# MILAB-IIT-CV/ATDN_vSLAM

Hardware: AMD Instinct MI355X
Metric: frame-pairs/sec, KITTI 1241x376 odometry inference at 1/2/4/8 MI355X (higher is better)
Workload: dtype f32 via 3xf16 split MFMA (fp32 accumulate); 1 GPU; KITTI seq-03-shaped 376x1241 uint8 frames (resident in HBM) resized to 376x1232, GMA flow 12 GRU iters + CLVO head -> 6-DoF trajectory (BASELINE configs[1]); streams_per_gpu=2, gru_iters=12, parallelism=pairs sharded x1, one all-gather of 512-d features, replicated LSTM scan

## Files before the change

atdn_vslam_amd/_lib.py:

```python
import ctypes as C
import os

_HERE = os.path.dirname(os.path.abspath(__file__))
LIB_PATH = os.environ.get("ATDN_LIB_PATH") or os.path.join(_HERE, "libatdn_hip.so")

_f32p = C.POINTER(C.c_float)
_i64p = C.POINTER(C.c_int64)
_vp = C.c_void_p

SIGNATURES = {
    "atdn_version": (C.c_int, []),
    "atdn_last_error": (C.c_char_p, []),
    "atdn_gma_create": (C.c_int, [C.POINTER(_vp), C.c_int, C.c_int, C.c_int, C.c_int]),
    "atdn_gma_set_low_latency": (C.c_int, [_vp, C.c_int]),
    "atdn_gma_load": (C.c_int, [_vp, C.c_char_p, _vp, _i64p, C.c_int]),
    "atdn_gma_finalize": (C.c_int, [_vp]),
    "atdn_gma_forward": (C.c_int, [_vp, _vp, _vp, C.c_int, C.c_int, _vp, _vp, _vp, _vp]),
    "atdn_gma_forward_predictions": (C.c_int, [_vp, _vp, _vp, C.c_int, C.c_int, _vp, _vp, _vp]),
    "atdn_gma_forward_sequence": (C.c_int, [_vp, _vp, C.c_int, C.c_int, _vp, _vp, _vp, _vp]),
    "atdn_gma_forward_sequence_continued": (C.c_int, [_vp, _vp, C.c_int, C.c_int, _vp, _vp, _vp, _vp]),
    "atdn_gma_debug_read": (C.c_long, [_vp, C.c_char_p, _vp, C.c_long, _vp]),
    "atdn_gma_profile": (C.c_int, [_vp, C.c_int, C.c_int, C.c_int, _f32p, _vp]),
    "atdn_gma_profile_mode": (C.c_int, [_vp, C.c_int, C.c_int, C.c_int, C.c_int, _f32p, _vp]),
    "atdn_gma_set_range_probe": (C.c_int, [_vp, C.c_int]),
# ... 45 lines not shown
    "atdn_flow_two_view_depth": (C.c_int, [_vp, _vp, _vp, C.c_int, C.c_int, C.c_int, C.c_double, C.c_double, C.c_double, C.c_double,
                                           C.c_double, C.c_double, C.c_double, _vp, _vp, _vp]),
    "atdn_flow_two_view_depth_host": (C.c_int, [_vp, _vp, _vp, C.c_int, C.c_int, C.c_int, C.c_double, C.c_double, C.c_double,
                                                C.c_double, C.c_double, C.c_double, C.c_double, _vp, _vp]),
    "atdn_depth_backproject": (C.c_int, [_vp, C.c_int, C.c_int, C.c_int, C.c_double, C.c_double, C.c_double, C.c_double, _vp, _vp]),
    "atdn_flow_track_step": (C.c_int, [_vp, _vp, _vp, _vp, C.c_int, C.c_int, C.c_int, _vp, _vp, _vp, C.c_double, C.c_double, C.c_double,
                                       C.c_double, C.c_double, C.c_double, C.c_double, _vp, _vp, _vp]),
    "atdn_flow_track_step_host": (C.c_int, [_vp, _vp, _vp, _vp, C.c_int, C.c_int, C.c_int, _vp, _vp, _vp, C.c_double, C.c_double,
                                            C.c_double, C.c_double, C.c_double, C.c_double, C.c_double, _vp, _vp]),
    "atdn_map_search": (C.c_int, [_vp, C.c_int, C.c_int, _vp, C.c_int, C.c_int, _vp, _vp, _vp]),
    "atdn_map_gather_images_u8": (C.c_int, [_vp, C.c_int, C.c_long, _vp, C.c_int, _vp, _vp]),
    "atdn_corr_lookup": (C.c_int, [_vp, _vp, _vp, _vp, C.c_int, C.c_int, C.c_int, _vp, _vp, C.c_int, _vp]),
    "atdn_corr_pyramid": (C.c_int, [_vp, _vp, C.c_int, C.c_int, C.c_int, C.c_int, _vp, _vp, _vp, _vp, _vp]),
    "atdn_corr_lookup_bricks": (C.c_int, [_vp, _vp, C.c_int, C.c_int, C.c_int, C.c_int, _vp, _vp, _vp, _vp, _vp, _vp, _vp, _vp,
                                          _vp, _vp]),
    "atdn_conv2d_nhwc": (C.c_int, [_vp, C.c_int, C.c_int, C.c_int, C.c_int, _vp, _vp, C.c_int, C.c_int, C.c_int,
                                   C.c_int, C.c_int, C.c_int, C.c_int, _vp, _vp]),
    "atdn_conv2d_nhwc_sf": (C.c_int, [_vp, C.c_int, C.c_int, C.c_int, C.c_int, _vp, _vp, C.c_int, C.c_int, C.c_int,
                                      C.c_int, C.c_int, C.c_int, _vp, _vp]),
    "atdn_conv2d_nhwc_sf_epi": (C.c_int, [_vp, C.c_int, C.c_int, C.c_int, C.c_int, _vp, _vp, C.c_int, C.c_int, C.c_int,
                                      C.c_int, C.c_int, C.c_int, C.c_int, _vp, _vp]),
}

GMA_STAGES = ("fnet", "corr", "pool", "cnet", "attention", "lookup", "motion_encoder", "aggregate", "gru_zr", "gru_q",
              "flow_head", "mask", "gru_ctx", "attn_logits", "agg_vt", "convc1", "gru_zr_v", "gru_q_v")

_lib = None


def lib():
# ... 37 lines not shown
```

atdn_vslam_amd/csrc/capi.hip:

```cpp
#include "../../include/atdn_hip.h"

#include <cmath>
#include <cstring>

#include "clvo.h"
#include "gma.h"
#include "vae.h"
#include "clvo_train.h"
#include "train_kernels.h"
#include "frontend.h"
#include "conv_sf.h"
#include "epilogues_sf.h"
#include "flow_args.h"
#include "flow_consistency_host.h"
#include "flow_track_host.h"
#include "two_view_host.h"
#include "warm_start_host.h"

namespace atdn {
extern template TileChoice conv_dispatch<MODE_TAP, EpiBias<ACT_NONE>>(const ConvShape&, EpiBias<ACT_NONE>, hipStream_t);
extern template TileChoice conv_dispatch<MODE_TAP, EpiBias<ACT_RELU>>(const ConvShape&, EpiBias<ACT_RELU>, hipStream_t);
extern template TileChoice conv_dispatch<MODE_ROW, EpiBias<ACT_NONE>>(const ConvShape&, EpiBias<ACT_NONE>, hipStream_t);
extern template TileChoice conv_dispatch<MODE_ROW, EpiBias<ACT_RELU>>(const ConvShape&, EpiBias<ACT_RELU>, hipStream_t);
extern template TileChoice conv_dispatch<MODE_TAP, EpiScale>(const ConvShape&, EpiScale, hipStream_t);
// ... 429 lines not shown
  bp.N = N; bp.NPB = brick_pixel_blocks(N);
  DeviceBuf f1, f2, plain[3], fbrick[4], pyr[4], scratch, outsf;
  DeviceBuf* all[] = {&f1, &f2, &plain[0], &plain[1], &plain[2], &fbrick[0], &fbrick[1], &fbrick[2], &fbrick[3],
                      &pyr[0], &pyr[1], &pyr[2], &pyr[3], &scratch, &outsf};
  WeightArena A;
  try {
    sf_counter_attach();
    f1.alloc(n8 * 256); f2.alloc(n8 * 256);
    launch_to_sf(fmap1, f1.p, n8, 256, st);
    launch_to_sf(fmap2, f2.p, n8, 256, st);
    float* rowmajor[4] = {pyr0, pyr1, pyr2, pyr3};
    int pH[4], pW[4];
    for (int l = 0; l < 4; ++l) {
      pH[l] = H8 >> l; pW[l] = W8 >> l;
      bp.H[l] = pH[l]; bp.W[l] = pW[l]; bp.BW[l] = cdiv(pW[l], 8); bp.BH[l] = cdiv(pH[l], 4); bp.NB[l] = bp.BW[l] * bp.BH[l] * 32;
      const float* src = f2.p;
      long src_sb = (long)N * 256;
      if (l > 0) {
        const float* prev = l == 1 ? f2.p : plain[l - 2].p;
        const long prev_sb = l == 1 ? (long)N * 256 : (long)pH[l - 1] * pW[l - 1] * 256;
        src_sb = (long)pH[l] * pW[l] * 256;
        plain[l - 1].alloc((long)B * src_sb);
        launch_pool_features_sf(prev, B, pH[l - 1], pW[l - 1], 256, prev_sb, plain[l - 1].p, src_sb, st);
        src = plain[l - 1].p;
      }
      fbrick[l].alloc((long)B * bp.NB[l] * 256);
      launch_brick_rows(src, src_sb, B, pH[l], pW[l], 256, fbrick[l].p, (long)bp.NB[l] * 256, st);
      pyr[l].alloc((long)B * bp.NPB * kBrickPixelBlock * bp.NB[l]);
      launch_corr_bricks(f1.p, (long)N * 256, fbrick[l].p, (long)bp.NB[l] * 256, B, N, bp.NB[l], 1.0f / sqrtf(256.0f), pyr[l].p, false, st);
      bp.base[l] = pyr[l].p;
      if (rowmajor[l]) launch_unbrick(pyr[l].p, bp.NB[l], N, pH[l], pW[l], n8, rowmajor[l], st);
    }
    if (samples) {
      outsf.alloc(n8 * 352);
      launch_lookup_bricks(bp, coords, n8, outsf.p, st);
      scratch.alloc(n8 * 352);
      launch_from_sf(outsf.p, scratch.p, n8, 352, st);
      ATDN_HIP(hipMemcpy2DAsync(samples, 324 * sizeof(float), scratch.p, 352 * sizeof(float), 324 * sizeof(float), (size_t)n8,
                                hipMemcpyDeviceToDevice, st));
    }
    if (cor1) {
      StateDict sd;
// ... 10 lines not shown
        launch_lookup_conv(bp, coords, n8, nullptr, L.wf16, L.wscale, L.b, csf.p, false, st);
        launch_from_sf(csf.p, cor1, n8, 256, st);
        ATDN_HIP(hipStreamSynchronize(st));
      } catch (...) { csf.release(); throw; }
      csf.release();
    }
    ATDN_HIP(hipStreamSynchronize(st));
  } catch (...) {
    (void)hipDeviceSynchronize();
    for (auto* b : all) b->release();
    A.release();
    throw;
  }
  for (auto* b : all) b->release();
  A.release();
  ATDN_API_END
}

int atdn_conv2d_nhwc(const float* src, int nimg, int H, int W, int Cin, const float* weight_host,
                     const float* bias_host, int Cout, int KH, int KW, int stride, int padH, int padW, int relu,
                     float* dst, void* stream) {
  ATDN_API_BEGIN
  ATDN_CHECK(src && weight_host && dst && nimg >= 1, "null argument");
  const bool row = (Cin == 4 || Cin == 16);
  ATDN_CHECK(row || Cin % 32 == 0, "Cin must be 4, 16 or a multiple of 32");
  StateDict sd;
  const int64_t ws[4] = {Cout, Cin, KH, KW};
  sd.put("c.weight", weight_host, ws, 4);
  std::vector<float> zb(Cout, 0.f);
  const int64_t bs[1] = {Cout};
// ... 136 lines not shown
```

atdn_vslam_amd/csrc/gma.h:

```cpp
#pragma once
#include <vector>
#include <map>
#include <memory>

#include "attention.h"
#include "conv_dispatch.h"
#include "kernels.h"
#include "range_probe.h"
#include "weights.h"

namespace atdn {

struct EncoderWeights {
  PackedConv stem;
  struct Block { PackedConv c1, c2, ds; bool has_ds = false; } blk[6];
  PackedConv head;
};

class DeviceBuf {
 public:
  float* p = nullptr;
  long n = 0;
  void alloc(long count) {
    n = count;
// ... 74 lines not shown
  WeightArena arena_;
  bool ready_ = false;
  bool use_graph_ = true;
  EncoderWeights fnet_, cnet_;
  PackedConv convc1_, convc2_, convf1_, convf2_, convm_, to_v_, to_qk_;
  long convf1_sf_off_ = -1;
  float convf1_wscale_ = 1.f;
  float fh2_mul_ = 1.f;
  long fh2_w32_off_ = -1;
  DeviceBuf fhG_;
  PackedConv gru_zr_[2], gru_q_[2], fh1_, fh2_, mask0_, mask2_;
  PackedConv gru_zr_ctx_[2], gru_q_ctx_[2];
  const float* gamma_ = nullptr;
  long gamma_off_ = -1;

  DeviceBuf img4_, enc_[4], scratch_, pcnt_, fin_, fmap_, psum_, pm2_, mean_[3], rstd_[3];
  DeviceBuf pyr_[4], h_[2], x_, qk_, attn_, vT_, corrfeat_, cor1_, corflo_, flo1_, z_, rh_, fh_, mask_;
  DeviceBuf coords1_, flow4_, pre_zr_[2], pre_q_[2];
  int pyrH_[4], pyrW_[4];
  size_t ws_bytes_ = 0;

  struct Timer;
  Timer* timer_ = nullptr;
  void mark(int stage, hipStream_t st);

  hipStream_t cap_stream_ = nullptr;
  std::map<std::pair<int, int>, hipGraphExec_t> graphs_;
};

}
```

atdn_vslam_amd/csrc/gma.hip:

```cpp
#include "gma.h"
#include "small_convs.h"
#include "conv_sf.h"
#include "epilogues_sf.h"

namespace atdn { const float* zero_line(); }

namespace atdn {

extern template TileChoice conv_dispatch<MODE_TAP, EpiBias<ACT_NONE>>(const ConvShape&, EpiBias<ACT_NONE>, hipStream_t);
extern template TileChoice conv_dispatch<MODE_TAP, EpiBias<ACT_RELU>>(const ConvShape&, EpiBias<ACT_RELU>, hipStream_t);
extern template TileChoice conv_dispatch<MODE_ROW, EpiBias<ACT_RELU>>(const ConvShape&, EpiBias<ACT_RELU>, hipStream_t);
extern template TileChoice conv_dispatch<MODE_TAP, EpiBiasStats>(const ConvShape&, EpiBiasStats, hipStream_t);
extern template TileChoice conv_dispatch<MODE_ROW, EpiBiasStats>(const ConvShape&, EpiBiasStats, hipStream_t);
extern template TileChoice conv_dispatch<MODE_TAP, EpiBiasReluAddRelu>(const ConvShape&, EpiBiasReluAddRelu, hipStream_t);
extern template TileChoice conv_dispatch<MODE_TAP, EpiContextSplit>(const ConvShape&, EpiContextSplit, hipStream_t);
extern template TileChoice conv_dispatch<MODE_TAP, EpiScale>(const ConvShape&, EpiScale, hipStream_t);
extern template TileChoice conv_dispatch<MODE_TAP, EpiQK>(const ConvShape&, EpiQK, hipStream_t);
extern template TileChoice conv_dispatch<MODE_TAP, EpiStoreT>(const ConvShape&, EpiStoreT, hipStream_t);
extern template TileChoice conv_dispatch<MODE_TAP, EpiAggregate>(const ConvShape&, EpiAggregate, hipStream_t);
extern template TileChoice conv_dispatch<MODE_TAP, EpiGruZR>(const ConvShape&, EpiGruZR, hipStream_t);
extern template TileChoice conv_dispatch<MODE_TAP, EpiGruQ>(const ConvShape&, EpiGruQ, hipStream_t);
extern template TileChoice conv_dispatch<MODE_TAP, EpiFlowDelta>(const ConvShape&, EpiFlowDelta, hipStream_t);

extern template TileChoice conv_dispatch<MODE_ROW, SfBias<ACT_RELU>>(const ConvShape&, SfBias<ACT_RELU>, hipStream_t);
// ... 125 lines not shown
  ATDN_HIP(hipStreamWaitEvent(to, e, 0));
}

void GmaNet::set_low_latency(bool on) {
  ATDN_CHECK(!ready_, "set_low_latency: call it before finalize() (the workspace and the captured graphs depend on it)");
  low_latency_ = on;
}

GmaNet::~GmaNet() {
  DeviceGuard dg(dev_);
  (void)hipDeviceSynchronize();
  for (auto& kv : graphs_) (void)hipGraphExecDestroy(kv.second);
  if (cap_stream_) (void)hipStreamDestroy(cap_stream_);
  if (par_stream_) (void)hipStreamDestroy(par_stream_);
  for (auto& e : par_events_) (void)hipEventDestroy(e);
  DeviceBuf* all[] = {&img4_, &enc_[0], &enc_[1], &enc_[2], &enc_[3], &scratch_, &pcnt_, &fin_, &fmap_, &psum_, &pm2_, &mean_[0], &mean_[1], &mean_[2], &rstd_[0],
                      &rstd_[1], &rstd_[2], &pyr_[0], &pyr_[1], &pyr_[2], &pyr_[3], &h_[0], &h_[1], &x_, &qk_, &attn_, &vT_,
                      &corrfeat_, &cor1_, &corflo_, &flo1_, &z_, &rh_, &fh_, &mask_, &coords1_, &flow4_, &pre_zr_[0],
                      &pre_zr_[1], &pre_q_[0], &pre_q_[1], &rowmax_, &rinv_,
                      &fbrick_[0], &fbrick_[1], &fbrick_[2], &fbrick_[3], &fplain_[0], &fplain_[1], &fplain_[2], &coords_used_, &fhG_,
                      &attn_part_, &enc2_[0], &enc2_[1], &enc2_[2], &enc2_[3]};
  for (auto* b : all) b->release();
  if (probe_slots_) (void)hipFree(probe_slots_);
  arena_.release();
}

void GmaNet::set_probe(bool on) {
  ATDN_CHECK(!on || precision == 0,
             "the range probe needs an exact-fp32 handle (ATDN_PRECISION_F32): only that path writes every intermediate tensor "
             "as plain fp32 and never clamps; the split-f16 / f16 paths store range-limited values and fuse some tensors away");
  probe_ = on;
// ... 104 lines not shown
  resolve_encoder(arena_, fnet_);
  resolve_encoder(arena_, cnet_);
  for (PackedConv* L : {&convc1_, &convc2_, &convf1_, &convf2_, &convm_, &to_v_, &to_qk_, &gru_zr_[0], &gru_zr_[1],
                        &gru_q_[0], &gru_q_[1], &fh1_, &fh2_, &mask0_, &mask2_})
    resolve(arena_, *L);
  if (sf) for (PackedConv* L : {&gru_zr_ctx_[0], &gru_zr_ctx_[1], &gru_q_ctx_[0], &gru_q_ctx_[1]}) resolve(arena_, *L);
  gamma_ = arena_.dev(gamma_off_);

  const int B = maxB;
  const int H2 = conv_out(H, 7, 2, 3), W2 = conv_out(W, 7, 2, 3);
  const long n8 = (long)B * N;
  img4_.alloc(2L * B * H * W * 4);
  for (int i = 0; i < (sf ? 4 : 3); ++i) enc_[i].alloc(2L * B * H2 * W2 * 64);
  fmap_.alloc(2L * B * N * 256);
  const long groups = (long)cdiv(H2 * W2, 64) * 4 + 8;
  psum_.alloc(2L * B * groups * 128); pm2_.alloc(2L * B * groups * 128); pcnt_.alloc(2L * B * groups); fin_.alloc(2L * B * 32 * 128 * 4 * 2);
  for (int i = 0; i < 3; ++i) { mean_[i].alloc(2L * B * 128); rstd_[i].alloc(2L * B * 128); }
  pyrH_[0] = H8; pyrW_[0] = W8;
  for (int l = 1; l < 4; ++l) { pyrH_[l] = pyrH_[l - 1] / 2; pyrW_[l] = pyrW_[l - 1] / 2; }
  ATDN_CHECK(pyrH_[3] >= 2 && pyrW_[3] >= 2, "frame too small for a 4-level pyramid");
  for (int l = 0; l < 4; ++l) {
    brickBW_[l] = cdiv(pyrW_[l], 8); brickBH_[l] = cdiv(pyrH_[l], 4); brickNB_[l] = brickBW_[l] * brickBH_[l] * 32;
    pyr_[l].alloc(classic_ ? n8 * pyrH_[l] * pyrW_[l] : (long)B * brick_pixel_blocks(N) * kBrickPixelBlock * brickNB_[l]);
  }
  if (sf) {
    for (int l = 0; l < 4; ++l) fbrick_[l].alloc((long)B * brickNB_[l] * 256);
    for (int l = 1; l < 4; ++l) fplain_[l - 1].alloc((long)B * pyrH_[l] * pyrW_[l] * 256);
    coords_used_.alloc(n8 * 2);
  }
  h_[0].alloc(n8 * 128); h_[1].alloc(n8 * 128); x_.alloc(n8 * XLD);
  const AttnGeom ag = attn_geom(B, N, ldN);
// ... 28 lines not shown
}

void GmaNet::run_encoder(const EncoderWeights& E, bool instance, int nimg, hipStream_t st, float** out_buf, int* outH,
                         int* outW) {
  int h = conv_out(H, 7, 2, 3), w = conv_out(W, 7, 2, 3);
  float* P = enc_[0].p; float* Q = enc_[1].p; float* R = enc_[2].p;
  auto stats_conv = [&](auto mode_tag, const PackedConv& L, const float* src, int ld, int ih, int iw, int stride,
                        int pad, float* dst, int slot) {
    constexpr int MODE = decltype(mode_tag)::value;
    ConvShape s = conv_shape(L, src, ld, (long)ih * iw * ld, nimg, ih, iw, stride, pad, pad);
    const int oh = conv_out(ih, L.KH, stride, pad), ow = conv_out(iw, L.KW, stride, pad);
    EpiBiasStats ep{L.b, dst, (long)oh * ow * L.N, L.N, psum_.p, pm2_.p, 0};
    TileChoice t = conv_dispatch<MODE>(s, ep, st);
    const int groups = cdiv(oh * ow, t.BM) * (t.BM / 32);
    ATDN_CHECK((long)nimg * groups * L.N <= psum_.n, "statistics scratch too small");
    launch_in_finalize_cnt(psum_.p, pm2_.p, nullptr, nimg, groups, oh * ow, L.N, 1e-5f, mean_[slot].p, rstd_[slot].p,
                           reinterpret_cast<double*>(fin_.p), st);
  };
  using TapT = std::integral_constant<int, MODE_TAP>;
  using RowT = std::integral_constant<int, MODE_ROW>;
  auto pr = [&](int bi, const char* leaf, bool limited, const float* p, long pixels, int ch) {
    if (!probe_) return;
    std::string name = instance ? "fnet." : "cnet.";
    if (bi >= 0) name += "layer" + std::to_string(bi / 2 + 1) + "." + std::to_string(bi % 2);
    probe(name + leaf, limited, p, (long)nimg * pixels, ch, ch, st);
  };

  if (instance) {
    stats_conv(RowT{}, E.stem, img4_.p, 4, H, W, 2, 3, P, 0);
    pr(-1, "conv1.raw", false, P, (long)h * w, 64);
    launch_in_apply(P, mean_[0].p, rstd_[0].p, nullptr, nullptr, nullptr, nimg, (long)h * w, 64, st);
  } else {
// ... 183 lines not shown
  const float* images = img4_.p + (long)first_img * H * W * 4;
  int h = conv_out(H, 7, 2, 3), w = conv_out(W, 7, 2, 3);
  DeviceBuf* eb = bufs ? bufs : enc_;
  float* X = eb[0].p; float* R = eb[1].p; float* Y = eb[2].p; float* O = eb[3].p;
  auto stats_sf = [&](const PackedConv& L, const float* src, int ld, int ih, int iw, int stride, int pad, float* dst,
                      int slot, int in_slot = -1) {
    ConvShape s = conv_shape(L, src, ld, (long)ih * iw * ld, nimg, ih, iw, stride, pad, pad);
    if (in_slot >= 0) { s.in_mean = mean_[in_slot].p; s.in_rstd = rstd_[in_slot].p; }
    const int oh = conv_out(ih, L.KH, stride, pad), ow = conv_out(iw, L.KW, stride, pad);
    EpiBiasStats ep{L.b, dst, (long)oh * ow * L.N, L.N, psum_.p, pm2_.p, 0, pcnt_.p};
    TileChoice t = conv_sf_dispatch(s, L.wscale, ep, st);
    const int groups = t.groups_per_img;
    ATDN_CHECK((long)nimg * groups * L.N <= psum_.n && (long)nimg * groups <= pcnt_.n, "statistics scratch too small");
    if (t.counted)
      launch_in_finalize_cnt(psum_.p, pm2_.p, pcnt_.p, nimg, groups, oh * ow, L.N, 1e-5f, mean_[slot].p,
                             rstd_[slot].p, reinterpret_cast<double*>(fin_.p), st);
    else
      launch_in_finalize_cnt(psum_.p, pm2_.p, nullptr, nimg, groups, oh * ow, L.N, 1e-5f, mean_[slot].p, rstd_[slot].p,
                             reinterpret_cast<double*>(fin_.p), st);
  };
  const bool stem_raw = instance && norm_on_load_;
  if (stem_raw) {
    const int groups = stem_sf_groups(h, w);
    ATDN_CHECK((long)nimg * groups * 64 <= psum_.n && (long)nimg * groups <= pcnt_.n, "statistics scratch too small");
    launch_stem_sf(3, images, nimg, H, W, E.stem.wf, E.stem.wscale, E.stem.b, X, psum_.p, pm2_.p, pcnt_.p, nullptr, nullptr, st);
    launch_in_finalize_cnt(psum_.p, pm2_.p, pcnt_.p, nimg, groups, h * w, 64, 1e-5f, mean_[2].p, rstd_[2].p,
                           reinterpret_cast<double*>(fin_.p), st);
  } else if (instance) {
    const int groups = stem_sf_groups(h, w);
    ATDN_CHECK((long)nimg * groups * 64 <= psum_.n && (long)nimg * groups <= pcnt_.n, "statistics scratch too small");
    launch_stem_sf(1, images, nimg, H, W, E.stem.wf, E.stem.wscale, E.stem.b, nullptr, psum_.p, pm2_.p, pcnt_.p, nullptr,
                   nullptr, st);
    launch_in_finalize_cnt(psum_.p, pm2_.p, pcnt_.p, nimg, groups, h * w, 64, 1e-5f, mean_[0].p, rstd_[0].p,
                           reinterpret_cast<double*>(fin_.p), st);
    launch_stem_sf(2, images, nimg, H, W, E.stem.wf, E.stem.wscale, E.stem.b, X, nullptr, nullptr, nullptr, mean_[0].p,
                   rstd_[0].p, st);
  } else {
    launch_stem_sf(0, images, nimg, H, W, E.stem.wf, E.stem.wscale, E.stem.b, X, nullptr, nullptr, nullptr, nullptr,
                   nullptr, st);
  }
  int c = 64;
  for (int bi = 0; bi < 6; ++bi) {
    const auto& Bk = E.blk[bi];
    const int stride = Bk.has_ds ? 2 : 1;
    const int co = Bk.c1.N;
    const int oh = conv_out(h, 3, stride, 1), ow = conv_out(w, 3, stride, 1);
    const long ohw = (long)oh * ow;
    if (instance && norm_on_load_) {
      const bool raw_in = stem_raw && bi == 0;
// ... 93 lines not shown
}

void GmaNet::run_body_sf(int B, int iters, hipStream_t st) {
  float* f;
  const int nfeat = seq_ == 0 ? 2 * B : seq_ == 1 ? B + 1 : B;
  hipStream_t sB = par_ ? par_stream_ : st;
  if (par_) fork(st, sB);
  run_encoder_sf(fnet_, true, nfeat, st, &f, seq_ == 2 ? 1 : 0);
  ConvShape s = conv_shape(fnet_.head, f, 128, (long)N * 128, nfeat, H8, W8, 1, 0, 0);
  float* fdst = fmap_.p + (seq_ == 2 ? (long)N * 256 : 0);
  conv_sf_dispatch(s, fnet_.head.wscale, SfBias<ACT_NONE>{fnet_.head.b, fdst, (long)N * 256, 256}, st);
  mark(ST_FNET, st);

  const float* target = fmap_.p + (long)(seq_ ? 1 : B) * N * 256;
  for (int l = 0; l < 4; ++l) {
    const float* plain = target;
    long plain_sb = (long)N * 256;
    if (l > 0) {
      const float* prev = l == 1 ? target : fplain_[l - 2].p;
      const long prev_sb = l == 1 ? (long)N * 256 : (long)pyrH_[l - 1] * pyrW_[l - 1] * 256;
      plain_sb = (long)pyrH_[l] * pyrW_[l] * 256;
      launch_pool_features_sf(prev, B, pyrH_[l - 1], pyrW_[l - 1], 256, prev_sb, fplain_[l - 1].p, plain_sb, st);
      plain = fplain_[l - 1].p;
    }
    launch_brick_rows(plain, plain_sb, B, pyrH_[l], pyrW_[l], 256, fbrick_[l].p, (long)brickNB_[l] * 256, st);
    launch_corr_bricks(fmap_.p, (long)N * 256, fbrick_[l].p, (long)brickNB_[l] * 256, B, N, brickNB_[l], 1.0f / sqrtf(256.0f), pyr_[l].p,
                       sf_fast_mode(), st);
    if (l == 0) mark(ST_CORR, st);
  }
  mark(ST_POOL, st);

  run_encoder_sf(cnet_, false, B, sB, &f, 0, par_ ? enc2_ : nullptr);
  s = conv_shape(cnet_.head, f, 128, (long)N * 128, B, H8, W8, 1, 0, 0);
  conv_sf_dispatch(s, cnet_.head.wscale,
                   SfContextSplit{cnet_.head.b, h_[0].p, (long)N * 128, x_.p, (long)N * XLD, XLD}, sB);
  mark(ST_CNET, st);

  s = conv_shape(to_qk_, x_.p, XLD, (long)N * XLD, B, H8, W8, 1, 0, 0);
  conv_sf_dispatch(s, to_qk_.wscale, SfQK{1.0f / sqrtf(128.0f), 128, qk_.p, (long)N * 256, 256}, sB);
  {
// ... 218 lines not shown
```

atdn_vslam_amd/csrc/kernels.h:

```cpp
#pragma once
#include "common.h"

namespace atdn {

bool& sf_fast_mode();

struct PyramidLevels {
  const float* base[4];
  int H[4], W[4];
};

void launch_prep_images(const float* im1, const float* im2, int B, int H, int W, float* img4, hipStream_t st, int n2);

int stem_sf_groups(int Ho, int Wo);
void launch_stem_sf(int mode, const float* img4, int nimg, int H, int W, const float* wfrag, float wscale,
                    const float* bias, float* out_sf, float* part_sum, float* part_m2, float* part_cnt,
                    const float* mean, const float* rstd, hipStream_t st);

void launch_in_finalize_cnt(const float* part_sum, const float* part_m2, const float* part_cnt, int nimg,
                            int groups_per_img, int HW, int C, float eps, float* mean, float* rstd, double* scratch,
                            hipStream_t st);
void launch_in_apply(float* x, const float* mean, const float* rstd, const float* res, const float* rmean,
                     const float* rrstd, int nimg, long HW, int C, hipStream_t st);

void launch_avgpool(const float* src, int H, int W, float* dst, long rows, hipStream_t st);

void launch_lookup(const PyramidLevels& pyr, const float* coords1, long npix_total, float* out, int ldo,
                   hipStream_t st);

void launch_softmax_rows(float* x, long rows, int n, int ld, hipStream_t st);

void launch_init_coords(const float* flow_init, int B, int H8, int W8, float* coords1, float* flow4, float* xflow,
                        int ldx, hipStream_t st);

void launch_upsample(const float* mask, const float* flow4, int B, int H8, int W8, float* flow_low, float* flow_up,
                     hipStream_t st);
// ... 13 lines not shown
void launch_lstm_pipe(const LstmPipeArgs& a, hipStream_t st);
long lstm_scan_exchange_bytes();
bool lstm_scan_fits_device();
void launch_lstm_scan(const float* pre1, const float* Whh1, const float* bhh1, const float* Wlin, const float* blin,
                      const float* Wih2, const float* bih2, const float* Whh2, const float* bhh2, float* state, float* h2seq,
                      void* exchange, int T, hipStream_t st);
struct MlpHead { const float *w0, *b0, *w1, *b1, *w2; };
void launch_mlp_heads(const float* h2, int B, MlpHead rot, MlpHead tr, float* rot_out, float* tr_out, hipStream_t st);

void launch_to_sf(const float* src, float* dst, long rows, int C, hipStream_t st);
void launch_from_sf(const float* src, float* dst, long rows, int C, hipStream_t st);
void launch_in_apply_sf(const float* x, float* y, const float* mean, const float* rstd, const float* res,
                        const float* res_raw, const float* rmean, const float* rrstd, int nimg, long HW, int C,
                        hipStream_t st, bool res_relu = false);
void launch_pool_features_sf(const float* src, int nimg, int H, int W, int C, long sb, float* dst, long db, hipStream_t st);
void launch_init_coords_sf(const float* flow_init, int B, int H8, int W8, float* coords1, float* flow4, float* x,
                           int ldx, int cflow, hipStream_t st);

void launch_fill(float* p, long n, float v, hipStream_t st);

constexpr int kBrickPixelBlock = 64;
struct BrickPyramid {
  const float* base[4];
  int H[4], W[4], BW[4], BH[4], NB[4];
  int N;
  int NPB;
};
inline int brick_pixel_blocks(int N) { return 2 * ((N + 127) / 128); }
void launch_brick_rows(const float* src, long sb, int nimg, int H, int W, int C, float* dst, long db, hipStream_t st);
void launch_corr_bricks(const float* f1, long sb1, const float* f2b, long sb2, int B, int N, int NB, float scale, float* out,
// ... 8 lines not shown
```

atdn_vslam_amd/csrc/kernels.hip:

```cpp
#include "kernels.h"
#include "sf.h"

namespace atdn {

bool& sf_fast_mode() {
  static thread_local bool fast = false;
  return fast;
}

__device__ __forceinline__ float wave_sum(float v) {
#pragma unroll
  for (int o = 32; o > 0; o >>= 1) v += __shfl_xor(v, o);
  return v;
}
__device__ __forceinline__ float wave_max(float v) {
#pragma unroll
  for (int o = 32; o > 0; o >>= 1) v = fmaxf(v, __shfl_xor(v, o));
  return v;
}
template <bool MAX>
__device__ __forceinline__ float block_reduce(float v, float* sm) {
  v = MAX ? wave_max(v) : wave_sum(v);
  __syncthreads();
  if ((threadIdx.x & 63) == 0) sm[threadIdx.x >> 6] = v;
// ... 63 lines not shown
  const int i = blockIdx.x * blockDim.x + threadIdx.x;
  if (i >= nimg * C) return;
  const int img = i / C, c = i - img * C;
  double n = 0.0, s1 = 0.0, sq = 0.0, m2 = 0.0;
  for (int z = 0; z < FIN_SPLIT; ++z) {
    const double* p = part + (((long)img * FIN_SPLIT + z) * C + c) * 4;
    n += p[0]; s1 += p[1]; sq += p[2]; m2 += p[3];
  }
  const double mu = n > 0.0 ? s1 / n : 0.0;
  const double between = n > 0.0 ? fmax(sq - s1 * s1 / n, 0.0) : 0.0;
  const float mu_f = (float)mu, rs_f = (float)(1.0 / sqrt((m2 + between) / (double)HW + (double)eps));
  mean[i] = mu_f;
  rstd[i] = rs_f;
  sf_report(!(fabsf(mu_f) <= 3.0e38f) | !(rs_f <= 3.0e38f));
}
void launch_in_finalize_cnt(const float* part_sum, const float* part_m2, const float* part_cnt, int nimg,
                            int groups_per_img, int HW, int C, float eps, float* mean, float* rstd, double* scratch,
                            hipStream_t st) {
  hipLaunchKernelGGL(in_finalize_cnt_kernel, dim3(cdiv(C, 64), nimg, FIN_SPLIT), dim3(1024), 0, st, part_sum, part_m2,
                     part_cnt, groups_per_img, C, HW, scratch);
  ATDN_HIP(hipGetLastError());
  hipLaunchKernelGGL(in_finalize_merge_kernel, dim3(cdiv(nimg * C, 128)), dim3(128), 0, st, scratch, nimg, HW, C, eps,
                     mean, rstd);
  ATDN_HIP(hipGetLastError());
}

__global__ void in_apply_kernel(float4* __restrict__ x, const float* __restrict__ mean, const float* __restrict__ rstd,
                                const float4* __restrict__ res, const float* __restrict__ rmean,
                                const float* __restrict__ rrstd, long per_img4, int C, long total4) {
  for (long i = (long)blockIdx.x * blockDim.x + threadIdx.x; i < total4; i += (long)gridDim.x * blockDim.x) {
    const long img = i / per_img4;
    const int c = (int)((i * 4) % C);
    const float* mu = mean + img * C + c;
// ... 549 lines not shown
  const float* s = src + img * sb;
  const long p00 = ((long)(2 * y) * W + 2 * x) * C;
  const float4 a = sf_load4(s, p00, 4 * cq), b = sf_load4(s, p00 + C, 4 * cq);
  const float4 c = sf_load4(s, p00 + (long)W * C, 4 * cq), d = sf_load4(s, p00 + (long)W * C + C, 4 * cq);
  const float4 o = make_float4((((a.x + b.x) + c.x) + d.x) * 0.25f, (((a.y + b.y) + c.y) + d.y) * 0.25f,
                               (((a.z + b.z) + c.z) + d.z) * 0.25f, (((a.w + b.w) + c.w) + d.w) * 0.25f);
  sf_store4(dst + img * db, (long)po * C, 4 * cq, o);
}
void launch_pool_features_sf(const float* src, int nimg, int H, int W, int C, long sb, float* dst, long db, hipStream_t st) {
  ATDN_CHECK(C % 32 == 0, "sf tensors need C % 32 == 0");
  const long total = (long)nimg * (H / 2) * (W / 2) * (C / 4);
  hipLaunchKernelGGL(pool_features_sf_kernel, dim3((unsigned)cdivl(total, 256)), dim3(256), 0, st, src, H, W, C, sb, dst, db, total);
  ATDN_HIP(hipGetLastError());
}

__global__ void init_coords_sf_kernel(const float* __restrict__ flow_init, int B, int H8, int W8,
                                      float* __restrict__ coords1, float* __restrict__ flow4, float* __restrict__ x,
                                      int ldx, int cflow) {
  const long N = (long)H8 * W8;
  const long i = (long)blockIdx.x * blockDim.x + threadIdx.x;
  if (i >= B * N) return;
  const long img = i / N;
  const int m = (int)(i - img * N);
  const float x0 = (float)(m % W8), y0 = (float)(m / W8);
  float fx = 0.f, fy = 0.f;
  if (flow_init) { fx = flow_init[(img * 2 + 0) * N + m]; fy = flow_init[(img * 2 + 1) * N + m]; }
  const float cx = x0 + fx, cy = y0 + fy;
  coords1[i * 2 + 0] = cx;
  coords1[i * 2 + 1] = cy;
  const float flx = cx - x0, fly = cy - y0;
// ... 14 lines not shown
```

include/atdn_hip.h:

```cpp
#ifndef ATDN_HIP_H
#define ATDN_HIP_H

#include <stddef.h>
#include <stdint.h>

#ifdef __cplusplus
extern "C" {
#endif

typedef struct atdn_gma atdn_gma;
typedef struct atdn_clvo atdn_clvo;
typedef struct atdn_vae atdn_vae;
typedef struct atdn_clvo_trainer atdn_clvo_trainer;

int atdn_version(void);
const char* atdn_last_error(void);


#define ATDN_PRECISION_F32 0
#define ATDN_PRECISION_SPLIT_F16 1
#define ATDN_PRECISION_F16 2
int atdn_gma_create(atdn_gma** out, int H, int W, int max_batch, int precision);

int atdn_gma_set_low_latency(atdn_gma* h, int on);
// ... 123 lines not shown
int atdn_map_search(const float* bank, int K, int D, const float* queries, int Q, int topk, float* dist, int* idx, void* stream);

int atdn_map_gather_images_u8(const uint8_t* bank, int K, long plane_bytes, const int* index_host, int n, float* out, void* stream);


int atdn_corr_lookup(const float* pyr0, const float* pyr1, const float* pyr2, const float* pyr3, int B, int H8,
                     int W8, const float* coords, float* out, int ldo, void* stream);

int atdn_corr_pyramid(const float* fmap1, const float* fmap2, int B, int H8, int W8, int C, float* pyr0, float* pyr1,
                      float* pyr2, float* pyr3, void* stream);

int atdn_corr_lookup_bricks(const float* fmap1, const float* fmap2, int B, int H8, int W8, int C, const float* coords,
                            float* pyr0, float* pyr1, float* pyr2, float* pyr3, float* samples,
                            const float* convc1_weight_host, const float* convc1_bias_host, float* cor1, void* stream);

int atdn_conv2d_nhwc(const float* src, int nimg, int H, int W, int Cin, const float* weight_host,
                     const float* bias_host, int Cout, int KH, int KW, int stride, int padH, int padW, int relu,
                     float* dst, void* stream);

int atdn_conv2d_nhwc_sf(const float* src, int nimg, int H, int W, int Cin, const float* weight_host,
                        const float* bias_host, int Cout, int KH, int KW, int stride, int padH, int padW, float* dst,
                        void* stream);
int atdn_conv2d_nhwc_sf_epi(const float* src, int nimg, int H, int W, int Cin, const float* weight_host,
                            const float* bias_host, int Cout, int KH, int KW, int stride, int padH, int padW, int sf_store,
                            float* dst, void* stream);

#ifdef __cplusplus
}
#endif
#endif
// ... 1 lines not shown
```

Baseline: 424.7 frame-pairs/s.

## Fuse pyramid pooling with brick relayout and make instance-norm finalize single-pass

Pyramid levels 1-3 now come from one kernel that average-pools the feature map and writes both the plain pooled map and the bricked layout, replacing a pool launch followed by a separate brick-rows pass. Instance-norm statistics finalize moves from a two-kernel path with a double scratch buffer to one kernel. That kernel reduces the partial sums per channel slab through wave shuffles and shared memory inside a block. The old paths stay reachable through new test entry points. The gains are fewer launches and less re-reading of pooled features, at the cost of a different reduction order and per-block occupancy in finalize.

```diff
diff --git a/atdn_vslam_amd/_lib.py b/atdn_vslam_amd/_lib.py
--- a/atdn_vslam_amd/_lib.py
+++ b/atdn_vslam_amd/_lib.py
@@ -83,6 +83,8 @@
     "atdn_corr_pyramid": (C.c_int, [_vp, _vp, C.c_int, C.c_int, C.c_int, C.c_int, _vp, _vp, _vp, _vp, _vp]),
     "atdn_corr_lookup_bricks": (C.c_int, [_vp, _vp, C.c_int, C.c_int, C.c_int, C.c_int, _vp, _vp, _vp, _vp, _vp, _vp, _vp, _vp,
                                           _vp, _vp]),
+    "atdn_in_finalize": (C.c_int, [_vp, _vp, _vp, C.c_int, C.c_int, C.c_int, C.c_int, C.c_float, C.c_int, _vp, _vp, _vp]),
+    "atdn_pool_brick_levels": (C.c_int, [_vp, C.c_int, C.c_int, C.c_int, C.c_int, _vp, _vp, _vp, _vp, _vp, _vp, _vp]),
     "atdn_conv2d_nhwc": (C.c_int, [_vp, C.c_int, C.c_int, C.c_int, C.c_int, _vp, _vp, C.c_int, C.c_int, C.c_int,
                                    C.c_int, C.c_int, C.c_int, C.c_int, _vp, _vp]),
     "atdn_conv2d_nhwc_sf": (C.c_int, [_vp, C.c_int, C.c_int, C.c_int, C.c_int, _vp, _vp, C.c_int, C.c_int, C.c_int,
diff --git a/atdn_vslam_amd/csrc/capi.hip b/atdn_vslam_amd/csrc/capi.hip
--- a/atdn_vslam_amd/csrc/capi.hip
+++ b/atdn_vslam_amd/csrc/capi.hip
@@ -467,18 +467,17 @@
     for (int l = 0; l < 4; ++l) {
       pH[l] = H8 >> l; pW[l] = W8 >> l;
       bp.H[l] = pH[l]; bp.W[l] = pW[l]; bp.BW[l] = cdiv(pW[l], 8); bp.BH[l] = cdiv(pH[l], 4); bp.NB[l] = bp.BW[l] * bp.BH[l] * 32;
-      const float* src = f2.p;
-      long src_sb = (long)N * 256;
+      fbrick[l].alloc((long)B * bp.NB[l] * 256);
       if (l > 0) {
         const float* prev = l == 1 ? f2.p : plain[l - 2].p;
         const long prev_sb = l == 1 ? (long)N * 256 : (long)pH[l - 1] * pW[l - 1] * 256;
-        src_sb = (long)pH[l] * pW[l] * 256;
-        plain[l - 1].alloc((long)B * src_sb);
-        launch_pool_features_sf(prev, B, pH[l - 1], pW[l - 1], 256, prev_sb, plain[l - 1].p, src_sb, st);
-        src = plain[l - 1].p;
+        const long plain_sb = (long)pH[l] * pW[l] * 256;
+        plain[l - 1].alloc((long)B * plain_sb);
+        launch_pool_brick_features_sf(prev, B, pH[l - 1], pW[l - 1], 256, prev_sb, plain[l - 1].p, plain_sb, fbrick[l].p,
+                                      (long)bp.NB[l] * 256, st);
+      } else {
+        launch_brick_rows(f2.p, (long)N * 256, B, pH[l], pW[l], 256, fbrick[l].p, (long)bp.NB[l] * 256, st);
       }
-      fbrick[l].alloc((long)B * bp.NB[l] * 256);
-      launch_brick_rows(src, src_sb, B, pH[l], pW[l], 256, fbrick[l].p, (long)bp.NB[l] * 256, st);
       pyr[l].alloc((long)B * bp.NPB * kBrickPixelBlock * bp.NB[l]);
       launch_corr_bricks(f1.p, (long)N * 256, fbrick[l].p, (long)bp.NB[l] * 256, B, N, bp.NB[l], 1.0f / sqrtf(256.0f), pyr[l].p, false, st);
       bp.base[l] = pyr[l].p;
@@ -519,6 +518,67 @@
   }
   for (auto* b : all) b->release();
   A.release();
+  ATDN_API_END
+}
+
+int atdn_in_finalize(const float* part_sum, const float* part_m2, const float* part_cnt, int nimg, int groups, int HW, int C,
+                     float eps, int two_pass, float* mean, float* rstd, void* stream) {
+  ATDN_API_BEGIN
+  ATDN_CHECK(part_sum && part_m2 && mean && rstd && nimg >= 1 && groups >= 1 && HW >= 1 && C >= 1, "bad argument");
+  hipStream_t st = (hipStream_t)stream;
+  sf_counter_attach();
+  if (!two_pass) {
+    launch_in_finalize_cnt(part_sum, part_m2, part_cnt, nimg, groups, HW, C, eps, mean, rstd, st);
+    ATDN_HIP(hipStreamSynchronize(st));
+  } else {
+    DeviceBuf scratch;
+    try {
+      scratch.alloc((long)nimg * 32 * C * 4 * 2);
+      launch_in_finalize_two_pass(part_sum, part_m2, part_cnt, nimg, groups, HW, C, eps, mean, rstd,
+                                  reinterpret_cast<double*>(scratch.p), st);
+      ATDN_HIP(hipStreamSynchronize(st));
+    } catch (...) {
+      (void)hipDeviceSynchronize();
+      scratch.release();
+      throw;
+    }
+    scratch.release();
+  }
+  ATDN_API_END
+}
+
+int atdn_pool_brick_levels(const float* fmap, int B, int H8, int W8, int two_pass, float* plain1, float* plain2, float* plain3,
+                           float* brick1, float* brick2, float* brick3, void* stream) {
+  ATDN_API_BEGIN
+  ATDN_CHECK(fmap && plain1 && plain2 && plain3 && brick1 && brick2 && brick3 && B >= 1, "bad argument");
+  ATDN_CHECK((H8 >> 3) >= 1 && (W8 >> 3) >= 1, "map too small for four pyramid levels");
+  hipStream_t st = (hipStream_t)stream;
+  const long N = (long)H8 * W8;
+  DeviceBuf f;
+  try {
+    sf_counter_attach();
+    f.alloc(B * N * 256);
+    launch_to_sf(fmap, f.p, B * N, 256, st);
+    float* plain[3] = {plain1, plain2, plain3};
+    float* brick[3] = {brick1, brick2, brick3};
+    for (int l = 1; l < 4; ++l) {
+      const int h = H8 >> l, w = W8 >> l, ph = H8 >> (l - 1), pw = W8 >> (l - 1);
+      const float* prev = l == 1 ? f.p : plain[l - 2];
+      const long prev_sb = (long)ph * pw * 256, plain_sb = (long)h * w * 256, brick_sb = (long)cdiv(w, 8) * cdiv(h, 4) * 32 * 256;
+      if (!two_pass) {
+        launch_pool_brick_features_sf(prev, B, ph, pw, 256, prev_sb, plain[l - 1], plain_sb, brick[l - 1], brick_sb, st);
+      } else {
+        launch_pool_features_sf(prev, B, ph, pw, 256, prev_sb, plain[l - 1], plain_sb, st);
+        launch_brick_rows(plain[l - 1], plain_sb, B, h, w, 256, brick[l - 1], brick_sb, st);
+      }
+    }
+    ATDN_HIP(hipStreamSynchronize(st));
+  } catch (...) {
+    (void)hipDeviceSynchronize();
+    f.release();
+    throw;
+  }
+  f.release();
   ATDN_API_END
 }
 
diff --git a/atdn_vslam_amd/csrc/gma.h b/atdn_vslam_amd/csrc/gma.h
--- a/atdn_vslam_amd/csrc/gma.h
+++ b/atdn_vslam_amd/csrc/gma.h
@@ -112,7 +112,7 @@
   const float* gamma_ = nullptr;
   long gamma_off_ = -1;
 
-  DeviceBuf img4_, enc_[4], scratch_, pcnt_, fin_, fmap_, psum_, pm2_, mean_[3], rstd_[3];
+  DeviceBuf img4_, enc_[4], scratch_, pcnt_, fmap_, psum_, pm2_, mean_[3], rstd_[3];
   DeviceBuf pyr_[4], h_[2], x_, qk_, attn_, vT_, corrfeat_, cor1_, corflo_, flo1_, z_, rh_, fh_, mask_;
   DeviceBuf coords1_, flow4_, pre_zr_[2], pre_q_[2];
   int pyrH_[4], pyrW_[4];
diff --git a/atdn_vslam_amd/csrc/gma.hip b/atdn_vslam_amd/csrc/gma.hip
--- a/atdn_vslam_amd/csrc/gma.hip
+++ b/atdn_vslam_amd/csrc/gma.hip
@@ -163,7 +163,7 @@
   if (cap_stream_) (void)hipStreamDestroy(cap_stream_);
   if (par_stream_) (void)hipStreamDestroy(par_stream_);
   for (auto& e : par_events_) (void)hipEventDestroy(e);
-  DeviceBuf* all[] = {&img4_, &enc_[0], &enc_[1], &enc_[2], &enc_[3], &scratch_, &pcnt_, &fin_, &fmap_, &psum_, &pm2_, &mean_[0], &mean_[1], &mean_[2], &rstd_[0],
+  DeviceBuf* all[] = {&img4_, &enc_[0], &enc_[1], &enc_[2], &enc_[3], &scratch_, &pcnt_, &fmap_, &psum_, &pm2_, &mean_[0], &mean_[1], &mean_[2], &rstd_[0],
                       &rstd_[1], &rstd_[2], &pyr_[0], &pyr_[1], &pyr_[2], &pyr_[3], &h_[0], &h_[1], &x_, &qk_, &attn_, &vT_,
                       &corrfeat_, &cor1_, &corflo_, &flo1_, &z_, &rh_, &fh_, &mask_, &coords1_, &flow4_, &pre_zr_[0],
                       &pre_zr_[1], &pre_q_[0], &pre_q_[1], &rowmax_, &rinv_,
@@ -298,7 +298,7 @@
   for (int i = 0; i < (sf ? 4 : 3); ++i) enc_[i].alloc(2L * B * H2 * W2 * 64);
   fmap_.alloc(2L * B * N * 256);
   const long groups = (long)cdiv(H2 * W2, 64) * 4 + 8;
-  psum_.alloc(2L * B * groups * 128); pm2_.alloc(2L * B * groups * 128); pcnt_.alloc(2L * B * groups); fin_.alloc(2L * B * 32 * 128 * 4 * 2);
+  psum_.alloc(2L * B * groups * 128); pm2_.alloc(2L * B * groups * 128); pcnt_.alloc(2L * B * groups);
   for (int i = 0; i < 3; ++i) { mean_[i].alloc(2L * B * 128); rstd_[i].alloc(2L * B * 128); }
   pyrH_[0] = H8; pyrW_[0] = W8;
   for (int l = 1; l < 4; ++l) { pyrH_[l] = pyrH_[l - 1] / 2; pyrW_[l] = pyrW_[l - 1] / 2; }
@@ -357,8 +357,7 @@
     TileChoice t = conv_dispatch<MODE>(s, ep, st);
     const int groups = cdiv(oh * ow, t.BM) * (t.BM / 32);
     ATDN_CHECK((long)nimg * groups * L.N <= psum_.n, "statistics scratch too small");
-    launch_in_finalize_cnt(psum_.p, pm2_.p, nullptr, nimg, groups, oh * ow, L.N, 1e-5f, mean_[slot].p, rstd_[slot].p,
-                           reinterpret_cast<double*>(fin_.p), st);
+    launch_in_finalize_cnt(psum_.p, pm2_.p, nullptr, nimg, groups, oh * ow, L.N, 1e-5f, mean_[slot].p, rstd_[slot].p, st);
   };
   using TapT = std::integral_constant<int, MODE_TAP>;
   using RowT = std::integral_constant<int, MODE_ROW>;
@@ -572,25 +571,22 @@
     ATDN_CHECK((long)nimg * groups * L.N <= psum_.n && (long)nimg * groups <= pcnt_.n, "statistics scratch too small");
     if (t.counted)
       launch_in_finalize_cnt(psum_.p, pm2_.p, pcnt_.p, nimg, groups, oh * ow, L.N, 1e-5f, mean_[slot].p,
-                             rstd_[slot].p, reinterpret_cast<double*>(fin_.p), st);
+                             rstd_[slot].p, st);
     else
-      launch_in_finalize_cnt(psum_.p, pm2_.p, nullptr, nimg, groups, oh * ow, L.N, 1e-5f, mean_[slot].p, rstd_[slot].p,
-                             reinterpret_cast<double*>(fin_.p), st);
+      launch_in_finalize_cnt(psum_.p, pm2_.p, nullptr, nimg, groups, oh * ow, L.N, 1e-5f, mean_[slot].p, rstd_[slot].p, st);
   };
   const bool stem_raw = instance && norm_on_load_;
   if (stem_raw) {
     const int groups = stem_sf_groups(h, w);
     ATDN_CHECK((long)nimg * groups * 64 <= psum_.n && (long)nimg * groups <= pcnt_.n, "statistics scratch too small");
     launch_stem_sf(3, images, nimg, H, W, E.stem.wf, E.stem.wscale, E.stem.b, X, psum_.p, pm2_.p, pcnt_.p, nullptr, nullptr, st);
-    launch_in_finalize_cnt(psum_.p, pm2_.p, pcnt_.p, nimg, groups, h * w, 64, 1e-5f, mean_[2].p, rstd_[2].p,
-                           reinterpret_cast<double*>(fin_.p), st);
+    launch_in_finalize_cnt(psum_.p, pm2_.p, pcnt_.p, nimg, groups, h * w, 64, 1e-5f, mean_[2].p, rstd_[2].p, st);
   } else if (instance) {
     const int groups = stem_sf_groups(h, w);
     ATDN_CHECK((long)nimg * groups * 64 <= psum_.n && (long)nimg * groups <= pcnt_.n, "statistics scratch too small");
     launch_stem_sf(1, images, nimg, H, W, E.stem.wf, E.stem.wscale, E.stem.b, nullptr, psum_.p, pm2_.p, pcnt_.p, nullptr,
                    nullptr, st);
-    launch_in_finalize_cnt(psum_.p, pm2_.p, pcnt_.p, nimg, groups, h * w, 64, 1e-5f, mean_[0].p, rstd_[0].p,
-                           reinterpret_cast<double*>(fin_.p), st);
+    launch_in_finalize_cnt(psum_.p, pm2_.p, pcnt_.p, nimg, groups, h * w, 64, 1e-5f, mean_[0].p, rstd_[0].p, st);
     launch_stem_sf(2, images, nimg, H, W, E.stem.wf, E.stem.wscale, E.stem.b, X, nullptr, nullptr, nullptr, mean_[0].p,
                    rstd_[0].p, st);
   } else {
@@ -714,16 +710,14 @@
 
   const float* target = fmap_.p + (long)(seq_ ? 1 : B) * N * 256;
   for (int l = 0; l < 4; ++l) {
-    const float* plain = target;
-    long plain_sb = (long)N * 256;
     if (l > 0) {
       const float* prev = l == 1 ? target : fplain_[l - 2].p;
       const long prev_sb = l == 1 ? (long)N * 256 : (long)pyrH_[l - 1] * pyrW_[l - 1] * 256;
-      plain_sb = (long)pyrH_[l] * pyrW_[l] * 256;
-      launch_pool_features_sf(prev, B, pyrH_[l - 1], pyrW_[l - 1], 256, prev_sb, fplain_[l - 1].p, plain_sb, st);
-      plain = fplain_[l - 1].p;
+      launch_pool_brick_features_sf(prev, B, pyrH_[l - 1], pyrW_[l - 1], 256, prev_sb, fplain_[l - 1].p,
+                                    (long)pyrH_[l] * pyrW_[l] * 256, fbrick_[l].p, (long)brickNB_[l] * 256, st);
+    } else {
+      launch_brick_rows(target, (long)N * 256, B, pyrH_[0], pyrW_[0], 256, fbrick_[0].p, (long)brickNB_[0] * 256, st);
     }
-    launch_brick_rows(plain, plain_sb, B, pyrH_[l], pyrW_[l], 256, fbrick_[l].p, (long)brickNB_[l] * 256, st);
     launch_corr_bricks(fmap_.p, (long)N * 256, fbrick_[l].p, (long)brickNB_[l] * 256, B, N, brickNB_[l], 1.0f / sqrtf(256.0f), pyr_[l].p,
                        sf_fast_mode(), st);
     if (l == 0) mark(ST_CORR, st);
diff --git a/atdn_vslam_amd/csrc/kernels.h b/atdn_vslam_amd/csrc/kernels.h
--- a/atdn_vslam_amd/csrc/kernels.h
+++ b/atdn_vslam_amd/csrc/kernels.h
@@ -18,8 +18,10 @@
                     const float* mean, const float* rstd, hipStream_t st);
 
 void launch_in_finalize_cnt(const float* part_sum, const float* part_m2, const float* part_cnt, int nimg,
-                            int groups_per_img, int HW, int C, float eps, float* mean, float* rstd, double* scratch,
-                            hipStream_t st);
+                            int groups_per_img, int HW, int C, float eps, float* mean, float* rstd, hipStream_t st);
+void launch_in_finalize_two_pass(const float* part_sum, const float* part_m2, const float* part_cnt, int nimg,
+                                 int groups_per_img, int HW, int C, float eps, float* mean, float* rstd, double* scratch,
+                                 hipStream_t st);
 void launch_in_apply(float* x, const float* mean, const float* rstd, const float* res, const float* rmean,
                      const float* rrstd, int nimg, long HW, int C, hipStream_t st);
 
@@ -63,6 +65,8 @@
                         const float* res_raw, const float* rmean, const float* rrstd, int nimg, long HW, int C,
                         hipStream_t st, bool res_relu = false);
 void launch_pool_features_sf(const float* src, int nimg, int H, int W, int C, long sb, float* dst, long db, hipStream_t st);
+void launch_pool_brick_features_sf(const float* src, int nimg, int H, int W, int C, long sb, float* plain, long pb,
+                                   float* brick, long bb, hipStream_t st);
 void launch_init_coords_sf(const float* flow_init, int B, int H8, int W8, float* coords1, float* flow4, float* x,
                            int ldx, int cflow, hipStream_t st);
 
diff --git a/atdn_vslam_amd/csrc/kernels.hip b/atdn_vslam_amd/csrc/kernels.hip
--- a/atdn_vslam_amd/csrc/kernels.hip
+++ b/atdn_vslam_amd/csrc/kernels.hip
@@ -101,9 +101,98 @@
   rstd[i] = rs_f;
   sf_report(!(fabsf(mu_f) <= 3.0e38f) | !(rs_f <= 3.0e38f));
 }
+constexpr int FIN_CH = 8;
+constexpr int FIN_K = FIN_CH / 2;
+constexpr int FIN_P = 16 / FIN_K;
+template <bool CNT>
+__global__ __launch_bounds__(1024) void in_finalize_kernel(const float* __restrict__ ps, const float* __restrict__ pm2,
+                                                           const float* __restrict__ pc, int groups, int C, int HW,
+                                                           float eps, float* __restrict__ mean,
+                                                           float* __restrict__ rstd) {
+  static_assert(FIN_K * FIN_P == 16 && (64 / FIN_CH) % FIN_P == 0, "a slab's threads share a wave");
+  __shared__ double s_z[FIN_SPLIT][FIN_CH][4];
+  const int img = blockIdx.x, lane = threadIdx.x & 63;
+  const int cl = lane % FIN_CH, c = blockIdx.y * FIN_CH + cl;
+  const int t = (threadIdx.x >> 6) * (64 / FIN_CH) + lane / FIN_CH;
+  const int z = t / FIN_P, part = t % FIN_P;
+  const int per = (groups + FIN_SPLIT - 1) / FIN_SPLIT;
+  const int g0 = z * per, g1 = min(groups, g0 + per);
+  double n = 0.0, s1[FIN_K], sq[FIN_K], m2[FIN_K];
+#pragma unroll
+  for (int k = 0; k < FIN_K; ++k) { s1[k] = 0.0; sq[k] = 0.0; m2[k] = 0.0; }
+  if (c < C) {
+    const float* s = ps + (long)img * groups * C;
+    const float* m = pm2 + (long)img * groups * C;
+    const float* cn = pc + (long)img * groups;
+    for (int gb = g0 + part * FIN_K; gb < g1; gb += 16) {
+      float sv[FIN_K], mv[FIN_K], cv[FIN_K];
+#pragma unroll
+      for (int k = 0; k < FIN_K; ++k) {
+        const int g = min(gb + k, g1 - 1);
+        const unsigned o = (unsigned)g * (unsigned)C + (unsigned)c;
+        sv[k] = s[o];
+        mv[k] = m[o];
+        cv[k] = CNT ? cn[g] : (float)max(0, min(32, HW - g * 32));
+      }
+#pragma unroll
+      for (int k = 0; k < FIN_K; ++k) {
+        const bool live = gb + k < g1 && cv[k] > 0.f;
+        const float cnt = live ? cv[k] : 32.f;
+        double r = 0.03125;
+        if (cnt != 32.f) r = 1.0 / (double)cnt;
+        const double sg = live ? (double)sv[k] : 0.0;
+        n += live ? (double)cnt : 0.0;
+        s1[k] += sg;
+        sq[k] += sg * sg * r;
+        m2[k] += live ? (double)mv[k] : 0.0;
+      }
+    }
+  }
+  double an = n, a1 = 0.0, aq = 0.0, a2 = 0.0;
+#pragma unroll
+  for (int k = 0; k < FIN_K; ++k) { a1 += s1[k]; aq += sq[k]; a2 += m2[k]; }
+#pragma unroll
+  for (int j = 1; j < FIN_P; ++j) {
+    const int lower = (lane - FIN_CH) & 63;
+    double bn = __shfl(an, lower) + n, b1 = __shfl(a1, lower), bq = __shfl(aq, lower), b2 = __shfl(a2, lower);
+#pragma unroll
+    for (int k = 0; k < FIN_K; ++k) { b1 += s1[k]; bq += sq[k]; b2 += m2[k]; }
+    if (part == j) { an = bn; a1 = b1; aq = bq; a2 = b2; }
+  }
+  if (part == FIN_P - 1) {
+    double* o = s_z[z][cl];
+    o[0] = an; o[1] = a1; o[2] = aq; o[3] = a2;
+  }
+  __syncthreads();
+  if (threadIdx.x < FIN_CH && c < C) {
+    double tn = 0.0, ts1 = 0.0, tsq = 0.0, tm2 = 0.0;
+#pragma unroll 4
+    for (int k = 0; k < FIN_SPLIT; ++k) {
+      const double* p = s_z[k][cl];
+      tn += p[0]; ts1 += p[1]; tsq += p[2]; tm2 += p[3];
+    }
+    const double mu = tn > 0.0 ? ts1 / tn : 0.0;
+    const double between = tn > 0.0 ? fmax(tsq - ts1 * ts1 / tn, 0.0) : 0.0;
+    const float mu_f = (float)mu, rs_f = (float)(1.0 / sqrt((tm2 + between) / (double)HW + (double)eps));
+    mean[(long)img * C + c] = mu_f;
+    rstd[(long)img * C + c] = rs_f;
+    sf_report(!(fabsf(mu_f) <= 3.0e38f) | !(rs_f <= 3.0e38f));
+  }
+}
 void launch_in_finalize_cnt(const float* part_sum, const float* part_m2, const float* part_cnt, int nimg,
-                            int groups_per_img, int HW, int C, float eps, float* mean, float* rstd, double* scratch,
-                            hipStream_t st) {
+                            int groups_per_img, int HW, int C, float eps, float* mean, float* rstd, hipStream_t st) {
+  const dim3 grid(nimg, cdiv(C, FIN_CH));
+  if (part_cnt)
+    hipLaunchKernelGGL(in_finalize_kernel<true>, grid, dim3(1024), 0, st, part_sum, part_m2, part_cnt, groups_per_img, C, HW,
+                       eps, mean, rstd);
+  else
+    hipLaunchKernelGGL(in_finalize_kernel<false>, grid, dim3(1024), 0, st, part_sum, part_m2, part_cnt, groups_per_img, C, HW,
+                       eps, mean, rstd);
+  ATDN_HIP(hipGetLastError());
+}
+void launch_in_finalize_two_pass(const float* part_sum, const float* part_m2, const float* part_cnt, int nimg,
+                                 int groups_per_img, int HW, int C, float eps, float* mean, float* rstd, double* scratch,
+                                 hipStream_t st) {
   hipLaunchKernelGGL(in_finalize_cnt_kernel, dim3(cdiv(C, 64), nimg, FIN_SPLIT), dim3(1024), 0, st, part_sum, part_m2,
                      part_cnt, groups_per_img, C, HW, scratch);
   ATDN_HIP(hipGetLastError());
@@ -683,6 +772,42 @@
   ATDN_HIP(hipGetLastError());
 }
 
+__global__ void pool_brick_features_sf_kernel(const float* __restrict__ src, int H, int W, int C, long sb,
+                                              float* __restrict__ plain, long pb, float* __restrict__ brick, long bb, int BW,
+                                              long total) {
+  const long i = (long)blockIdx.x * blockDim.x + threadIdx.x;
+  if (i >= total) return;
+  const int Ho = H / 2, Wo = W / 2, c4 = C / 4;
+  const int cq = (int)(i % c4);
+  const long row = i / c4;
+  const long per_img = bb / C;
+  const long img = row / per_img;
+  const int n = (int)(row - img * per_img);
+  const int bk = n >> 5, within = n & 31;
+  const int y = (bk / BW) * 4 + (within >> 3), x = (bk % BW) * 8 + (within & 7);
+  float4 o = make_float4(0.f, 0.f, 0.f, 0.f);
+  if (y < Ho && x < Wo) {
+    const float* s = src + img * sb;
+    const long p00 = ((long)(2 * y) * W + 2 * x) * C;
+    const float4 a = sf_load4(s, p00, 4 * cq), b = sf_load4(s, p00 + C, 4 * cq);
+    const float4 c = sf_load4(s, p00 + (long)W * C, 4 * cq), d = sf_load4(s, p00 + (long)W * C + C, 4 * cq);
+    o = make_float4((((a.x + b.x) + c.x) + d.x) * 0.25f, (((a.y + b.y) + c.y) + d.y) * 0.25f,
+                    (((a.z + b.z) + c.z) + d.z) * 0.25f, (((a.w + b.w) + c.w) + d.w) * 0.25f);
+    sf_store4(plain + img * pb, ((long)y * Wo + x) * C, 4 * cq, o);
+  }
+  sf_store4(brick + img * bb, (long)n * C, 4 * cq, o);
+}
+void launch_pool_brick_features_sf(const float* src, int nimg, int H, int W, int C, long sb, float* plain, long pb,
+                                   float* brick, long bb, hipStream_t st) {
+  ATDN_CHECK(C % 32 == 0 && bb % C == 0, "sf tensors need C % 32 == 0");
+  const int BW = (W / 2 + 7) / 8;
+  ATDN_CHECK(bb / C == (long)BW * ((H / 2 + 3) / 4) * 32, "pool_brick_features: the brick buffer does not fit the pooled map");
+  const long total = (long)nimg * (bb / C) * (C / 4);
+  hipLaunchKernelGGL(pool_brick_features_sf_kernel, dim3((unsigned)cdivl(total, 256)), dim3(256), 0, st, src, H, W, C, sb,
+                     plain, pb, brick, bb, BW, total);
+  ATDN_HIP(hipGetLastError());
+}
+
 __global__ void init_coords_sf_kernel(const float* __restrict__ flow_init, int B, int H8, int W8,
                                       float* __restrict__ coords1, float* __restrict__ flow4, float* __restrict__ x,
                                       int ldx, int cflow) {
diff --git a/include/atdn_hip.h b/include/atdn_hip.h
--- a/include/atdn_hip.h
+++ b/include/atdn_hip.h
@@ -161,6 +161,12 @@
                             float* pyr0, float* pyr1, float* pyr2, float* pyr3, float* samples,
                             const float* convc1_weight_host, const float* convc1_bias_host, float* cor1, void* stream);
 
+int atdn_in_finalize(const float* part_sum, const float* part_m2, const float* part_cnt, int nimg, int groups, int HW, int C,
+                     float eps, int two_pass, float* mean, float* rstd, void* stream);
+
+int atdn_pool_brick_levels(const float* fmap, int B, int H8, int W8, int two_pass, float* plain1, float* plain2, float* plain3,
+                           float* brick1, float* brick2, float* brick3, void* stream);
+
 int atdn_conv2d_nhwc(const float* src, int nimg, int H, int W, int Cin, const float* weight_host,
                      const float* bias_host, int Cout, int KH, int KW, int stride, int padH, int padW, int relu,
                      float* dst, void* stream);
```

Result: no change. 425.2 frame-pairs/s, median of 6 (+0.1%).
